# ishine/Prior-DiffuSE

Measured on AMD Instinct MI355X. Metric: enhanced-audio sec/sec (RTF), 6-step fast sampling, B=32, higher is better.
Workload: dtype f16x2; 1 GPU; B=32 x 4 s 16 kHz utterances per GPU, [B,2,401,161] spectrograms, GCRN prior + DiffUNet1 6-step sampling, STFT..ISTFT, seeded random weights; global_batch=32, frames=401, parallelism=batch-shard x1, graph=True, streams_per_gpu=1, batches_in_flight=3

## Files before the change

include/pdse.h:

```cpp
#ifndef PDSE_H
#define PDSE_H
#include <stdint.h>

#ifdef __cplusplus
extern "C" {
#endif

#define PDSE_ABI_VERSION 9

typedef void* pdse_stream_t;

enum pdse_act { PDSE_ACT_NONE = 0, PDSE_ACT_PRELU = 1, PDSE_ACT_ELU = 2, PDSE_ACT_SIGMOID = 3 };

enum pdse_epi {
  PDSE_EPI_LINEAR = 0,
  PDSE_EPI_GLU = 1,
  PDSE_EPI_BIGLU = 2
};

typedef struct pdse_src {
  const float* ptr;
  int64_t sb, sc, st, sf;
  int32_t C;
  int32_t act;
// ... 110 lines not shown
  int32_t reflect_own, pad_;
} pdse_wavprep_desc;

typedef struct pdse_ola_desc {
  const float* frames;
  const float* win2;
  const float* c;
  float* out;
  int32_t B, T, L, n_fft, hop, pad_;
  const int32_t* nframes;
  const int32_t* lens;
} pdse_ola_desc;

typedef struct pdse_qsample_desc {
  const float* label;
  const float* init;
  const float* noise;
  const float* a;
  const float* s;
  float* out;
  int64_t plane;
  int32_t B, mode;
} pdse_qsample_desc;

#define PDSE_MASKLOSS_BLOCKS 32
typedef struct pdse_maskloss_desc {
  const float* esti;
  const float* label;
  const int32_t* frames;
  double* partial;
  float* out;
  int32_t B, C, T, F;
} pdse_maskloss_desc;

typedef struct pdse_sigma_desc {
  const float* init;
  const float* a;
  float* out;
  float* maxbuf;
  int64_t plane;
  int32_t nplanes, pad_;
  const int32_t* valid;
} pdse_sigma_desc;

typedef struct pdse_ln_desc {
  const float* in;
  const float* gamma;
  const float* beta;
  float* out;
  int64_t osb, os_hi, os_lo, os_t;
  int32_t B, T, N, r;
  float eps;
  int32_t blk;
} pdse_ln_desc;

typedef struct pdse_lstm_desc {
  const float* gx;
  const float* whh;
  float* hT;
  float* cst;
  float* y;
  int64_t y_sb, y_st, y_su, y_sg;
  int32_t B, Bp, T, H, G, pad_;
} pdse_lstm_desc;

typedef struct pdse_glstm_desc {
  const float* gx1;
  const float* whh1;
  const float* wih2;
  const float* r2;
  const float* c2;
  const float* whh2;
  float* hT1;
  float* cst1;
  float* hT2;
  float* cst2;
  float* gx2;
  float* part;
  float* y;
  int64_t y_sb, y_st, y_su, y_sg;
  int32_t B, Bp, T, H, G;
  float eps;
  int32_t slices;
  int32_t pad_;
} pdse_glstm_desc;

typedef struct pdse_glstmp_desc {
  const float* gx1;
  const float* w1;
  const float* w2i;
  const float* w2h;
  const float* r2;
  const float* c2;
  unsigned long long* gran;
  int32_t* status;
  float* y;
  int64_t y_sb, y_st, y_su, y_sg;
  int32_t B, Bp, T, H, G;
  float eps;
} pdse_glstmp_desc;


typedef struct pdse_rowln_desc {
  const float* in;
  const float* gamma;
  const float* beta;
  const float* slope;
  float* out;
  int64_t out_sb;
  int32_t B, C, T, F;
  float eps;
  int32_t pad_;
} pdse_rowln_desc;

typedef struct pdse_dense_desc {
  float* D;
  const void* w;
  const float* bias;
  const float* gamma;
  const float* beta;
  const float* slope;
  int32_t B, T, F, G, tpad;
  int32_t g_in, cin;
  int32_t g_out;
  int32_t dil, np;
  float eps;
  int32_t wexp;
} pdse_dense_desc;

typedef struct pdse_rowlnb_desc {
  const float* in;
  const float* gamma;
  const float* beta;
  const float* slope;
  float* out;
  int64_t in_sb, in_sc, in_st;
  int64_t out_sb, out_sg, out_st;
  int32_t B, C, T, F;
  float eps;
  int32_t pad_;
} pdse_rowlnb_desc;

typedef struct pdse_chln_desc {
  const float* in;
  const float* gamma;
  const float* beta;
  float* out;
  int64_t plane;
  int32_t B, C;
  float eps;
  int32_t pad_;
} pdse_chln_desc;

typedef struct pdse_attn_desc {
  const float* qkv;
  float* out;
  int32_t B, T, F, E, heads, axis, pad0_, pad1_;
} pdse_attn_desc;

typedef struct pdse_gru_desc {
  const float* gx;
  const float* whh;
  const float* bhh;
  float* y;
  int32_t B, T, F, H, axis;
  int32_t split;
// ... 333 lines not shown
```

prior-diffuse_amd/_lib.py:

```python
import contextlib
import ctypes as C
import os

_HERE = os.path.dirname(os.path.abspath(__file__))
LIB_PATH = os.environ.get("PDSE_LIB") or os.path.join(_HERE, "libpdse.so")

ABI_VERSION = 9

ACT_NONE, ACT_PRELU, ACT_ELU, ACT_SIGMOID = 0, 1, 2, 3
EPI_LINEAR, EPI_GLU, EPI_BIGLU = 0, 1, 2
EW_DIV, EW_UPDATE, EW_UPDATE_FINAL, EW_COPY, EW_ADD_MUL = 0, 1, 2, 3, 4
(OP_GCONV, OP_TIME, OP_EW, OP_COMPAND, OP_WAVPREP, OP_OLA, OP_SIGMA, OP_LN, OP_LSTM,
 OP_ROWLN, OP_CHLN, OP_ATTN, OP_GRU, OP_GNCOMB, OP_AHAM, OP_QSAMPLE, OP_TRANSPOSE, OP_TCM, OP_CRM, OP_GCRNLAST,
 OP_MASKLOSS, OP_GLSTM, OP_TCM2, OP_BGLU, OP_PLANES, OP_GLSTMP, OP_TCM2S, OP_DENSE, OP_ROWLNB, OP_METRICS, OP_RESAMPLE, OP_RANGE) = range(32)
MASKLOSS_BLOCKS = 32

_fp = C.c_void_p
_i32, _i64, _f32 = C.c_int32, C.c_int64, C.c_float


class Src(C.Structure):
    _fields_ = [("ptr", _fp), ("sb", _i64), ("sc", _i64), ("st", _i64), ("sf", _i64),
                ("C", _i32), ("act", _i32), ("blk", _i32), ("pad_", _i32)]


class GconvDesc(C.Structure):
    _fields_ = [
        ("in0", Src), ("in1", Src),
        ("Tin", _i32), ("Fin", _i32),
        ("padrow", _fp), ("padrow_sb", _i64),
        ("taps", _fp), ("ntaps", _i32), ("sf_in", _i32),
        ("xf_scale0", _fp), ("xf_shift0", _fp), ("xf_scale1", _fp), ("xf_shift1", _fp),
        ("xf_slope0", _f32), ("xf_slope1", _f32), ("xf_mode", _i32), ("cin1", _i32),
        ("w0", _fp), ("w1", _fp), ("ksteps", _i32), ("Cout", _i32),
        ("bias0", _fp), ("bias1", _fp), ("bias0_sb", _i64), ("bias1_sb", _i64),
        ("epi", _i32), ("act", _i32), ("act_slope", _f32), ("C2", _i32),
        ("post_scale", _fp), ("post_shift", _fp),
        ("wlc", _fp), ("wrc", _fp), ("blc", _fp), ("brc", _fp), ("wc2", _fp), ("bc2", _fp),
        ("resid", _fp), ("out", _fp),
        ("out_sb", _i64), ("out_sc_hi", _i64), ("out_sc_lo", _i64), ("out_st", _i64),
        ("out_sf", _i64), ("out_off", _i64),
        ("out_cr", _i32), ("B", _i32), ("Tout", _i32), ("Fout", _i32),
        ("korder", _i32), ("ksteps1", _i32), ("w2", _fp), ("w3", _fp), ("p1mask", _i32), ("Fout1", _i32),
        ("nx_w", _fp), ("nx_bias", _fp * 3), ("nx_add", _fp * 3), ("nx_out", _fp * 3), ("nx_bias_sb", _i64 * 3),
        ("nx_sb", _i64 * 3), ("nx_sc", _i64 * 3), ("nx_st", _i64 * 3), ("nx_sf", _i64 * 3), ("nx_off", _i64 * 3),
        ("nx_n", _i32), ("nx_keep", _i32), ("nx_row0", _i32), ("wexp", _i32),
        ("bias0_t0", _fp), ("bias1_t0", _fp),
        ("tap_dt", _i32 * 12), ("tap_df", _i32 * 12), ("flat", _i32), ("pad_", _i32),
    ]


class TimeDesc(C.Structure):
    _fields_ = [("t", _fp), ("table", _fp), ("p1T", _fp), ("b1", _fp), ("p2T", _fp), ("b2", _fp),
                ("wfT", _fp), ("bf", _fp), ("out", _fp), ("temb", _fp),
                ("B", _i32), ("NF", _i32), ("max_steps", _i32), ("pad_", _i32)]


class EwDesc(C.Structure):
    _fields_ = [("a", _fp), ("b", _fp), ("c", _fp), ("out", _fp), ("n", _i64),
                ("s0", _f32), ("s1", _f32), ("s2", _f32), ("op", _i32)]


class CompandDesc(C.Structure):
    _fields_ = [("in_", _fp), ("out", _fp), ("plane", _i64), ("B", _i32), ("mode", _i32),
                ("out_sb", _i64), ("out_sc", _i64), ("out_st", _i64), ("F", _i32), ("pad_", _i32)]


class WavprepDesc(C.Structure):
    _fields_ = [("wav", _fp), ("xpad", _fp), ("c", _fp), ("lens", _fp),
                ("B", _i32), ("L", _i32), ("pad", _i32), ("normalize", _i32), ("reflect_own", _i32), ("pad_", _i32)]


class OlaDesc(C.Structure):
    _fields_ = [("frames", _fp), ("win2", _fp), ("c", _fp), ("out", _fp),
                ("B", _i32), ("T", _i32), ("L", _i32), ("n_fft", _i32), ("hop", _i32), ("pad_", _i32),
                ("nframes", _fp), ("lens", _fp)]


class SigmaDesc(C.Structure):
    _fields_ = [("init", _fp), ("a", _fp), ("out", _fp), ("maxbuf", _fp), ("plane", _i64),
                ("nplanes", _i32), ("pad_", _i32), ("valid", _fp)]


class LnDesc(C.Structure):
    _fields_ = [("in_", _fp), ("gamma", _fp), ("beta", _fp), ("out", _fp),
                ("osb", _i64), ("os_hi", _i64), ("os_lo", _i64), ("os_t", _i64),
                ("B", _i32), ("T", _i32), ("N", _i32), ("r", _i32), ("eps", _f32), ("blk", _i32)]


class LstmDesc(C.Structure):
    _fields_ = [("gx", _fp), ("whh", _fp), ("hT", _fp), ("cst", _fp), ("y", _fp),
                ("y_sb", _i64), ("y_st", _i64), ("y_su", _i64), ("y_sg", _i64),
                ("B", _i32), ("Bp", _i32), ("T", _i32), ("H", _i32), ("G", _i32), ("pad_", _i32)]


class GlstmDesc(C.Structure):
    _fields_ = [("gx1", _fp), ("whh1", _fp), ("wih2", _fp), ("r2", _fp), ("c2", _fp), ("whh2", _fp),
                ("hT1", _fp), ("cst1", _fp), ("hT2", _fp), ("cst2", _fp), ("gx2", _fp), ("part", _fp), ("y", _fp),
                ("y_sb", _i64), ("y_st", _i64), ("y_su", _i64), ("y_sg", _i64),
                ("B", _i32), ("Bp", _i32), ("T", _i32), ("H", _i32), ("G", _i32), ("eps", _f32), ("slices", _i32), ("pad_", _i32)]


class GlstmpDesc(C.Structure):
    _fields_ = [("gx1", _fp), ("w1", _fp), ("w2i", _fp), ("w2h", _fp), ("r2", _fp), ("c2", _fp), ("gran", _fp), ("status", _fp),
                ("y", _fp), ("y_sb", _i64), ("y_st", _i64), ("y_su", _i64), ("y_sg", _i64),
                ("B", _i32), ("Bp", _i32), ("T", _i32), ("H", _i32), ("G", _i32), ("eps", _f32)]


class RowlnDesc(C.Structure):
    _fields_ = [("in_", _fp), ("gamma", _fp), ("beta", _fp), ("slope", _fp), ("out", _fp), ("out_sb", _i64),
                ("B", _i32), ("C", _i32), ("T", _i32), ("F", _i32), ("eps", _f32), ("pad_", _i32)]


class DenseDesc(C.Structure):
    _fields_ = [("D", _fp), ("w", _fp), ("bias", _fp), ("gamma", _fp), ("beta", _fp), ("slope", _fp),
                ("B", _i32), ("T", _i32), ("F", _i32), ("G", _i32), ("tpad", _i32), ("g_in", _i32), ("cin", _i32), ("g_out", _i32),
                ("dil", _i32), ("np", _i32), ("eps", _f32), ("wexp", _i32)]


class RowlnbDesc(C.Structure):
    _fields_ = [("in_", _fp), ("gamma", _fp), ("beta", _fp), ("slope", _fp), ("out", _fp),
                ("in_sb", _i64), ("in_sc", _i64), ("in_st", _i64), ("out_sb", _i64), ("out_sg", _i64), ("out_st", _i64),
                ("B", _i32), ("C", _i32), ("T", _i32), ("F", _i32), ("eps", _f32), ("pad_", _i32)]


class ChlnDesc(C.Structure):
    _fields_ = [("in_", _fp), ("gamma", _fp), ("beta", _fp), ("out", _fp), ("plane", _i64),
                ("B", _i32), ("C", _i32), ("eps", _f32), ("pad_", _i32)]


class AttnDesc(C.Structure):
    _fields_ = [("qkv", _fp), ("out", _fp), ("B", _i32), ("T", _i32), ("F", _i32), ("E", _i32),
                ("heads", _i32), ("axis", _i32), ("pad0_", _i32), ("pad1_", _i32)]


class GruDesc(C.Structure):
    _fields_ = [("gx", _fp), ("whh", _fp), ("bhh", _fp), ("y", _fp),
                ("B", _i32), ("T", _i32), ("F", _i32), ("H", _i32), ("axis", _i32), ("split", _i32),
                ("x", _fp), ("wih", _fp), ("bih", _fp)]


class GncombDesc(C.Structure):
    _fields_ = [("base", _fp), ("row", _fp), ("col", _fp), ("g_row", _fp), ("b_row", _fp), ("g_col", _fp),
                ("b_col", _fp), ("stats", _fp), ("out", _fp), ("plane", _i64), ("B", _i32), ("C", _i32),
                ("k1", _f32), ("k2", _f32), ("eps", _f32), ("pad_", _i32)]


class AhamDesc(C.Structure):
    _fields_ = [("x", _fp * 4), ("w", _fp), ("means", _fp), ("out", _fp), ("plane", _i64),
                ("B", _i32), ("C", _i32), ("bias", _f32), ("pad_", _i32)]


class QsampleDesc(C.Structure):
    _fields_ = [("label", _fp), ("init", _fp), ("noise", _fp), ("a", _fp), ("s", _fp), ("out", _fp),
                ("plane", _i64), ("B", _i32), ("mode", _i32)]


class MasklossDesc(C.Structure):
    _fields_ = [("esti", _fp), ("label", _fp), ("frames", _fp), ("partial", _fp), ("out", _fp),
                ("B", _i32), ("C", _i32), ("T", _i32), ("F", _i32)]


class TransposeDesc(C.Structure):
    _fields_ = [("in_", _fp), ("out", _fp), ("N", _i32), ("R", _i32), ("Cc", _i32), ("pad_", _i32)]


class TcmDesc(C.Structure):
    _fields_ = [("x", _fp), ("h", _fp), ("x_out", _fp), ("h_out", _fp), ("wbr", _fp), ("bmain", _fp), ("bmask", _fp),
                ("xf", _fp), ("wc2", _fp), ("bc2", _fp), ("xf2", _fp), ("wn1", _fp), ("bn1", _fp),
                ("slope_main", _f32), ("slope_mask", _f32), ("slope2", _f32), ("dil", _i32), ("B", _i32), ("T", _i32),
                ("frames", _fp)]


class Tcm2Desc(C.Structure):
    _fields_ = [("x", _fp), ("x_out", _fp), ("hs", _fp), ("hs_out", _fp), ("wbr", _fp), ("wc2", _fp), ("wn1", _fp),
                ("par", _fp), ("slope2", _f32), ("slope_main_next", _f32), ("slope_mask_next", _f32),
                ("dil", _i32), ("B", _i32), ("T", _i32), ("mode", _i32), ("np", _i32), ("qexp", _i32 * 3),
                ("frames", _fp)]


TCM2S_MAX = 20


# ... 279 lines not shown
```

prior-diffuse_amd/csrc/lstm.hip:

```cpp
#include <hip/hip_runtime.h>
#include <stdio.h>
#include <stdint.h>
#include <stdlib.h>

#include "pdse.h"
#include "pdse_internal.h"

typedef float f32x16 __attribute__((ext_vector_type(16)));

__device__ __forceinline__ float sigm(float x) { return 1.0f / (1.0f + expf(-x)); }

template <int KPW>
__global__ __launch_bounds__(512) void lstm_step_kernel(const pdse_lstm_desc d, const int t, const int pp) {
  __shared__ float red[8][32][33];
  const int lane = threadIdx.x & 63, wave = threadIdx.x >> 6;
  const int col = lane & 31, h = lane >> 5;
  const int slice = blockIdx.x, g = blockIdx.y, bt = blockIdx.z;
  const int H = d.H, Bp = d.Bp, G = d.G;
  const float* hprev = d.hT + ((size_t)(pp * G + g) * H) * Bp + bt * 32;
  float* hnext = d.hT + ((size_t)((pp ^ 1) * G + g) * H) * Bp + bt * 32;
  const int KS = H / 2;
  const float* A = d.whh + ((size_t)(g * (H / 8) + slice) * KS) * 64 + lane;

  f32x16 acc;
#pragma unroll
  for (int r = 0; r < 16; ++r) acc[r] = 0.f;
  if (t > 0) {
    float av[KPW], bv[KPW];
    const int ks0 = wave * KPW;
#pragma unroll
    for (int i = 0; i < KPW; ++i) {
      av[i] = A[(size_t)(ks0 + i) * 64];
      bv[i] = hprev[(size_t)(2 * (ks0 + i) + h) * Bp + col];
    }
    __builtin_amdgcn_sched_barrier(0);
#pragma unroll
    for (int i = 0; i < KPW; ++i) acc = __builtin_amdgcn_mfma_f32_32x32x2f32(av[i], bv[i], acc, 0, 0, 0);
  }
  const int u = threadIdx.x >> 5 & 7, bb = threadIdx.x & 31;
  const int b = bt * 32 + bb;
  const int hu = slice * 8 + u;
  float gxv[4] = {0.f, 0.f, 0.f, 0.f};
  float c_old = 0.f;
  const size_t ci = ((size_t)g * H + hu) * Bp + b;
  if (threadIdx.x < 256) {
#pragma unroll
    for (int q = 0; q < 4; ++q) gxv[q] = d.gx[(((size_t)g * d.T + t) * (4 * H) + (size_t)q * H + hu) * Bp + b];
    if (t > 0) c_old = d.cst[ci];
  }
#pragma unroll
  for (int r = 0; r < 16; ++r) red[wave][(r & 3) + 8 * (r >> 2) + 4 * h][col] = acc[r];
  __syncthreads();
  if (threadIdx.x < 256) {
    float gate[4];
#pragma unroll
    for (int q = 0; q < 4; ++q) {
      const int i = q * 8 + u;
      float s = 0.f;
#pragma unroll
      for (int w = 0; w < 8; ++w) s += red[w][i][bb];
      gate[q] = s + gxv[q];
    }
    const float c = sigm(gate[1]) * c_old + sigm(gate[0]) * tanhf(gate[2]);
    const float hv = sigm(gate[3]) * tanhf(c);
    d.cst[ci] = c;
    hnext[(size_t)hu * Bp + bb] = hv;
    if (b < d.B) d.y[(int64_t)b * d.y_sb + (int64_t)t * d.y_st + (int64_t)hu * d.y_su + (int64_t)g * d.y_sg] = hv;
  }
}

int pdse_lstm_launch(const pdse_lstm_desc* d, hipStream_t s) {
  if (!d || !d->gx || !d->whh || !d->hT || !d->cst || !d->y) {
    pdse_set_error("lstm: null pointer");
    return 1;
  }
  if (d->B <= 0 || d->T <= 0 || d->G <= 0 || d->H != 512 || d->Bp % 32 != 0 || d->Bp < d->B) {
    pdse_set_error("lstm: bad sizes (H == 512 as in gcrn.py:9-16, Bp % 32 == 0, Bp >= B)");
    return 1;
  }
  const dim3 grid(d->H / 8, d->G, d->Bp / 32), block(512);
  for (int t = 0; t < d->T; ++t) hipLaunchKernelGGL(lstm_step_kernel<32>, grid, block, 0, s, *d, t, t & 1);
  return pdse_check_launch("lstm");
}

__device__ __forceinline__ float sigm_g(float x) { return 1.0f / (1.0f + expf(-x)); }

__device__ __forceinline__ size_t hidx(const int u, const int b, const int Bp) {
  return (((size_t)(u >> 3) * 2 + (u & 1)) * Bp + b) * 4 + ((u & 7) >> 1);
}

__device__ long long* g_trace_l = nullptr;
#define LSTAMP(i)                                                                                               \
  do {                                                                                                          \
    if (trace && lane == 0)                                                                                     \
      trace[((((size_t)blockIdx.z * gridDim.y + blockIdx.y) * gridDim.x + blockIdx.x) * 8 + wave) * 8 + (i)] =  \
          (i) == 0 ? wall_clock64() : clock64();                                                                \
  } while (0)

template <int NS>
__global__ __launch_bounds__(512) void glstm_wave_kernel(const pdse_glstm_desc d, const int s, const int stage_mask) {
  extern __shared__ __attribute__((aligned(16))) float lds_[];
  float (*red)[32 * NS][33] = reinterpret_cast<float (*)[32 * NS][33]>(lds_);
  float (*stat)[32][2] = reinterpret_cast<float (*)[32][2]>(lds_ + 8 * 32 * NS * 33);
  float (*gxs)[32][8 * NS] = reinterpret_cast<float (*)[32][8 * NS]>(lds_ + 8 * 32 * NS * 33 + 16 * 32 * 2);
  const int lane = threadIdx.x & 63, wave = threadIdx.x >> 6;
  const int col = lane & 31, h = lane >> 5;
  const int slice = blockIdx.x * NS, g = blockIdx.y;
  const int nbt = d.Bp >> 5;
  const int stage = blockIdx.z / nbt, bt = blockIdx.z - stage * nbt;
  const int t = s - stage;
  if (t < 0 || t >= d.T || !((stage_mask >> stage) & 1)) return;
#ifdef PDSE_DIAG
  long long* const trace = (s == d.T / 2) ? g_trace_l : nullptr;
#else
  long long* const trace = nullptr;
#endif
  LSTAMP(0);
  LSTAMP(1);
  const int H = d.H, Bp = d.Bp, G = d.G;
  const size_t hsz = (size_t)H * Bp;
  const int par = t & 1;

  const float* Aw;
  const float* hsrc0;
  const float* hsrc1;
  int kq0, kq1;
  bool skip = false;
  if (stage == 0) {
    Aw = d.whh1;
    hsrc0 = hsrc1 = d.hT1 + ((size_t)par * G + g) * hsz;
    kq0 = 0, kq1 = 32;
    skip = t == 0;
  } else if (stage == 1) {
    Aw = d.wih2;
    const float* base = d.hT1 + (size_t)((t + 1) & 1) * G * hsz;
    hsrc0 = base, hsrc1 = base + hsz;
    kq0 = kq1 = 32 * g;
  } else {
    Aw = d.whh2;
    hsrc0 = hsrc1 = d.hT2 + ((size_t)par * G + g) * hsz;
    kq0 = 0, kq1 = 32;
    skip = t == 0;
  }
  const float4* A4 = reinterpret_cast<const float4*>(Aw) + ((size_t)(g * (H / 8) + slice) * (H / 8)) * 64 + lane;

  f32x16 acc[NS];
#pragma unroll
  for (int n = 0; n < NS; ++n)
#pragma unroll
    for (int r = 0; r < 16; ++r) acc[n][r] = 0.f;
  if (!skip) {
    float4 av[NS][8], bv[8];
    const int q0 = wave * 8;
    const float* hs = q0 < 32 ? hsrc0 : hsrc1;
    const int kq = (q0 < 32 ? kq0 : kq1) + (q0 & 31);
    const float4* B4 = reinterpret_cast<const float4*>(hs) + ((size_t)kq * 2 + h) * Bp + bt * 32 + col;
    const float k0 = stage == 1 ? hsrc0[(size_t)(bt * 32 + col) * 4] : 0.f;
#pragma unroll
    for (int i = 0; i < 8; ++i) {
#pragma unroll
      for (int n = 0; n < NS; ++n) av[n][i] = A4[((size_t)n * (H / 8) + q0 + i) * 64];
      bv[i] = B4[(size_t)i * 2 * Bp];
    }
    __builtin_amdgcn_sched_barrier(0);
    if (stage == 1) {
#pragma unroll
      for (int i = 0; i < 8; ++i) bv[i].x -= k0, bv[i].y -= k0, bv[i].z -= k0, bv[i].w -= k0;
    }
    if (trace) {
      asm volatile("s_waitcnt vmcnt(0)" ::: "memory");
      LSTAMP(2);
    }
#pragma unroll
    for (int i = 0; i < 8; ++i) {
#pragma unroll
      for (int n = 0; n < NS; ++n) {
        acc[n] = __builtin_amdgcn_mfma_f32_32x32x2f32(av[n][i].x, bv[i].x, acc[n], 0, 0, 0);
        acc[n] = __builtin_amdgcn_mfma_f32_32x32x2f32(av[n][i].y, bv[i].y, acc[n], 0, 0, 0);
        acc[n] = __builtin_amdgcn_mfma_f32_32x32x2f32(av[n][i].z, bv[i].z, acc[n], 0, 0, 0);
        acc[n] = __builtin_amdgcn_mfma_f32_32x32x2f32(av[n][i].w, bv[i].w, acc[n], 0, 0, 0);
      }
    }
  }

  constexpr int NFIN = 256 * NS;
  const int uu = (threadIdx.x >> 5) & (8 * NS - 1), bb = threadIdx.x & 31;
  const int sl = uu >> 3, u = uu & 7;
  const int b = bt * 32 + bb;
  const int hu = (slice + sl) * 8 + u;
  float pre[4] = {0.f, 0.f, 0.f, 0.f};
  float4 gx4 = make_float4(0.f, 0.f, 0.f, 0.f);
  float c_old = 0.f;
  const size_t ci = ((size_t)g * H + hu) * Bp + b;
  if (threadIdx.x < NFIN) {
    if (stage == 0) {
      const int lq = threadIdx.x / (64 * NS), lb = (threadIdx.x / (2 * NS)) & 31, lu = (threadIdx.x & (2 * NS - 1)) * 4;
      gx4 = *reinterpret_cast<const float4*>(d.gx1 + (((size_t)g * d.T + t) * Bp + bt * 32 + lb) * (4 * H) + (size_t)lq * H + slice * 8 + lu);
      if (t > 0) c_old = d.cst1[ci];
    } else if (stage == 2) {
#pragma unroll
      for (int q = 0; q < 4; ++q) pre[q] = d.gx2[(((size_t)par * G + g) * (4 * H) + (size_t)q * H + hu) * Bp + b];
      if (t > 0) c_old = d.cst2[ci];
    }
  }
  float k0e = 0.f;
  if (stage == 1) {
    k0e = hsrc0[(size_t)b * 4];
    const int p = threadIdx.x >> 5;
    const float2* P2 = reinterpret_cast<const float2*>(d.part) + ((size_t)par * G * (H / 8)) * Bp + b;
    float2 pv[8];
    float s1 = 0.f, m2 = 0.f;
#pragma unroll
    for (int e = 0; e < 8; ++e) {
      pv[e] = P2[(size_t)(p * 8 + e) * Bp];
      s1 += pv[e].x;
    }
    const float mp = s1 * (1.0f / 64.0f);
#pragma unroll
    for (int e = 0; e < 8; ++e) {
      const float dv = pv[e].x * 0.125f - mp;
      m2 += pv[e].y + 8.0f * (dv * dv);
    }
    stat[p][bb][0] = s1;
    stat[p][bb][1] = m2;
  }
  LSTAMP(3);
#pragma unroll
  for (int n = 0; n < NS; ++n)
#pragma unroll
    for (int r = 0; r < 16; ++r) red[wave][32 * n + (r & 3) + 8 * (r >> 2) + 4 * h][col] = acc[n][r];
  if (stage == 0 && threadIdx.x < NFIN) {
    const int lq = threadIdx.x / (64 * NS), lb = (threadIdx.x / (2 * NS)) & 31, lu = (threadIdx.x & (2 * NS - 1)) * 4;
    *reinterpret_cast<float4*>(&gxs[lq][lb][lu]) = gx4;
  }
  __syncthreads();
  if (stage == 0 && threadIdx.x < NFIN) {
#pragma unroll
    for (int q = 0; q < 4; ++q) pre[q] = gxs[q][bb][uu];
  }
  LSTAMP(4);
  const bool fin = threadIdx.x < NFIN;
  float gate[4] = {0.f, 0.f, 0.f, 0.f};
  if (fin) {
#pragma unroll
    for (int q = 0; q < 4; ++q) {
      const int i = 32 * sl + q * 8 + u;
      float sum = 0.f;
#pragma unroll
      for (int w = 0; w < 8; ++w) sum += red[w][i][bb];
      gate[q] = sum;
    }
  }
  if (stage == 1) {
    if (!fin) return;
    double s1 = 0.0;
#pragma unroll
    for (int p = 0; p < 16; ++p) s1 += (double)stat[p][bb][0];
    const double n = (double)(G * H);
    const double mu = s1 / n;
    const float muf = (float)mu;
    float m2 = 0.f;
#pragma unroll
    for (int p = 0; p < 16; ++p) {
      const float dv = stat[p][bb][0] * (1.0f / 64.0f) - muf;
      m2 += stat[p][bb][1] + 64.0f * (dv * dv);
    }
    const double var = (double)m2 / n;
    const float rs = (float)(1.0 / sqrt(var + (double)d.eps));
    const float muk = (float)(mu - (double)k0e);
    float* out = d.gx2 + (((size_t)par * G + g) * (4 * H)) * Bp;
#pragma unroll
    for (int q = 0; q < 4; ++q) {
      const size_t row = (size_t)q * H + hu;
      out[row * Bp + b] = rs * (gate[q] - muk * d.r2[(size_t)g * 4 * H + row]) + d.c2[(size_t)g * 4 * H + row];
    }
    return;
  }
  float hv = 0.f;
  if (fin) {
#pragma unroll
    for (int q = 0; q < 4; ++q) gate[q] += pre[q];
    const float c = sigm_g(gate[1]) * c_old + sigm_g(gate[0]) * tanhf(gate[2]);
    hv = sigm_g(gate[3]) * tanhf(c);
    if (stage == 0) {
      d.cst1[ci] = c;
      d.hT1[((size_t)(par ^ 1) * G + g) * hsz + hidx(hu, b, Bp)] = hv;
      stat[uu][bb][0] = hv;
    } else {
      d.cst2[ci] = c;
      d.hT2[((size_t)(par ^ 1) * G + g) * hsz + hidx(hu, b, Bp)] = hv;
      if (b < d.B) d.y[(int64_t)b * d.y_sb + (int64_t)t * d.y_st + (int64_t)hu * d.y_su + (int64_t)g * d.y_sg] = hv;
    }
  }
  LSTAMP(5);
  if (stage != 0) return;
  __syncthreads();
  if (threadIdx.x < 32 * NS) {
    const int ps = threadIdx.x >> 5;
    float v[8];
    float s1 = 0.f, m2 = 0.f;
#pragma unroll
    for (int k = 0; k < 8; ++k) {
      v[k] = stat[8 * ps + k][bb][0];
      s1 += v[k];
    }
    const float m = s1 * 0.125f;
#pragma unroll
    for (int k = 0; k < 8; ++k) {
      const float e = v[k] - m;
      m2 += e * e;
    }
    float2* P2 = reinterpret_cast<float2*>(d.part) + (((size_t)par * G + g) * (H / 8) + slice + ps) * Bp + b;
    *P2 = make_float2(s1, m2);
  }
}


int pdse_glstm_launch(const pdse_glstm_desc* d, hipStream_t s) {
  if (!d || !d->gx1 || !d->whh1 || !d->wih2 || !d->r2 || !d->c2 || !d->whh2 || !d->hT1 || !d->cst1 || !d->hT2 ||
      !d->cst2 || !d->gx2 || !d->part || !d->y) {
    pdse_set_error("glstm: null pointer");
    return 1;
  }
  if (d->B <= 0 || d->T <= 0 || d->G != 2 || d->H != 512 || d->Bp % 32 != 0 || d->Bp < d->B || (d->Bp / 32) * 3 > 65535) {
    pdse_set_error("glstm: bad sizes (H == 512, G == 2 as in gcrn.py:9-16, Bp % 32 == 0, Bp >= B)");
    return 1;
  }
  if (d->slices < 0 || d->slices > 2) {
    pdse_set_error("glstm: slices is 0 / 1 (one slice of 8 units per workgroup) or 2");
    return 1;
  }
  const int NS = d->slices == 2 ? 2 : 1;
  const dim3 grid(d->H / 8 / NS, d->G, 3 * (d->Bp / 32)), block(512);
  const size_t lds = (size_t)(8 * 32 * NS * 33 + 16 * 32 * 2 + 4 * 32 * 8 * NS) * sizeof(float);
  static unsigned long long attr_mask = 0;
  if (NS == 2 && pdse_lds_attr((const void*)glstm_wave_kernel<2>, &attr_mask, "glstm lds attribute")) return 1;
  static const int mask = PDSE_DIAG_ENV("PDSE_GLSTM_MASK") ? atoi(PDSE_DIAG_ENV("PDSE_GLSTM_MASK")) : 7;
  static const bool tracing = PDSE_DIAG_ENV("PDSE_GLSTM_TRACE") != nullptr;
  static long long* tbuf = nullptr;
  const size_t nw = (size_t)grid.x * grid.y * grid.z * 8;
  if (tracing) {
    if (!tbuf) {
      (void)hipMalloc(&tbuf, nw * 64);
      (void)hipMemcpyToSymbol(HIP_SYMBOL(g_trace_l), &tbuf, sizeof(tbuf));
    }
    (void)hipMemsetAsync(tbuf, 0, nw * 64, s);
  }
  for (int st = 0; st < d->T + 2; ++st) {
    if (NS == 2) hipLaunchKernelGGL(glstm_wave_kernel<2>, grid, block, lds, s, *d, st, mask);
    else hipLaunchKernelGGL(glstm_wave_kernel<1>, grid, block, lds, s, *d, st, mask);
  }
  if (tracing) {
    (void)hipStreamSynchronize(s);
    long long* h = (long long*)malloc(nw * 64);
    (void)hipMemcpy(h, tbuf, nw * 64, hipMemcpyDeviceToHost);
    for (int stg = 0; stg < 3; ++stg) {
      double sum[8] = {0};
      long long w0 = -1, w1 = 0;
      size_t n = 0;
      const size_t per = nw / 3;
      for (size_t i = stg * per; i < (stg + 1) * per; ++i) {
        const long long* q = h + i * 8;
        if (!q[0]) continue;
        ++n;
        if (w0 < 0 || q[0] < w0) w0 = q[0];
        if (q[0] > w1) w1 = q[0];
        for (int k = 2; k < 6; ++k) sum[k] += q[k] ? (double)(q[k] - q[1]) : 0.0;
      }
      if (n) fprintf(stderr, "glstm trace stage %d (%zu waves): start spread %.2f us; cycles since wave start: loads landed %.0f, mfma issued %.0f, after barrier %.0f, end %.0f\n",
                     stg, n, (w1 - w0) * 0.01, sum[2] / n, sum[3] / n, sum[4] / n, sum[5] / n);
    }
    free(h);
  }
  return pdse_check_launch("glstm");
}
```

prior-diffuse_amd/nets.py:

```python
import ctypes as C

import numpy as np
import torch

from . import _lib as L
from . import packing as P

F0 = 161
BIG = 1 << 30

TAG_NONE, TAG_EPS_BLOCK, TAG_EPS_CONV1, TAG_TCM, TAG_PRIOR, TAG_LSTM, TAG_SIGNAL, TAG_EW = range(8)


class WeightBank:

    def __init__(self):
        self.items = {}
        self.keep = []
        self.owners = []

    def token(self, obj):
        if obj is None:
            return None
        for i, o in enumerate(self.owners):
# ... 802 lines not shown
                Fin = self._biconvglu_composed(step, src_x, src_i, o, ostr, nx)
            else:
                Fin = self._biconvglu(step, k, src_x, src_i, Fin, o, ostr, H=Hc, do_conv1=(k == 1 or not chained), nx=nx)
            if chained:
                Hc, Hn = Hn, Hc
            src_x, src_i = self.src(o, 64, *nchw(64, T, Fin)), None
        cur, nxt = self.en[4], self.tcm_a
        names = [("TCMs.%d.residual%d" % (i, j + 1), dil) for i in range(3) for j, dil in enumerate((1, 2, 4, 8, 16, 32))]
        if self.force_generic or not self.fused_tcm:
            for p, dil in names:
                self._residual(p, dil, cur, nxt)
                cur, nxt = nxt, (self.tcm_b if nxt is self.tcm_a else self.tcm_a)
        elif self.split_bf16 and self.split_tcm:
            hcur, hnxt = self.tcm_hs
            self._residual_split(None, 1, cur, None, None, hcur, names[0][0], mode=1)
            self._tcm_stack = [] if self.use_tcm_stack else None
            for n, (p, dil) in enumerate(names):
                p_next = names[n + 1][0] if n + 1 < len(names) else None
                self._residual_split(p, dil, cur, nxt, hcur, hnxt, p_next)
                cur, nxt = nxt, (self.tcm_b if nxt is self.tcm_a else self.tcm_a)
                hcur, hnxt = hnxt, hcur
            if self._tcm_stack:
                sd_ = L.Tcm2sDesc()
                for n, blk in enumerate(self._tcm_stack):
                    sd_.blk[n] = blk
                sd_.n = len(self._tcm_stack)
                sd_.flags, sd_.status = self.tcm_flags.data_ptr(), self.tcm_status.data_ptr()
                self.add(sd_, TAG_TCM)
            self._tcm_stack = None
        else:
            hcur, hnxt = self.tcm_h, self.tcm_g
            self._tcm_conv1(names[0][0], cur, hcur)
            for n, (p, dil) in enumerate(names):
                p_next = names[n + 1][0] if n + 1 < len(names) else None
                self._residual_fused(p, dil, cur, nxt, hcur, hnxt, p_next)
                cur, nxt = nxt, (self.tcm_b if nxt is self.tcm_a else self.tcm_a)
                hcur, hnxt = hnxt, hcur
        tcm_out = cur
        if self._plane_stage("dec"):
            self._decoders_planes(step, tcm_out, out)
            return out
        for di, de in enumerate(("de_real", "de_imag")):
            in0 = self.src(tcm_out, 64, 256 * T, 4 * T, 1, T)
            Fin = 4
            Hc, Hn = self.H, self.H2
            for n, k in enumerate((5, 4, 3, 2, 1)):
                skip = self.en[k - 1]
                if k == 5:
                    in1 = self.src(skip, 64, 256 * T, 4 * T, 1, T)
                else:
                    in1 = self.src(skip, 64, *nchw(64, T, self.ENC_F[k]))
                p = "%s.de%d.0" % (de, k)
                if k > 1:
                    o, ooff = self.dec[n & 1], 0
                    fn = lambda Fo: nchw_out(64, T, Fo)
                    bn, pr = "%s.de%d.2" % (de, k), "%s.de%d.3.weight" % (de, k)
                else:
                    o, ooff = out, di * T * F0
                    fn = lambda Fo: nchw_out(2, T, Fo)
                    bn, pr = None, None
                nx = None
                if chained and k > 1:
                    Fo = 2 * (Fin - 1) + 3
                    wn = lambda de=de, k=k: self.w("%s.de%d.0.conv1.weight" % (de, k - 1))[:, :, 0, 0].T[:, :64]
                    nx = dict(keep=False, row0=-1, tiles=[dict(wfn=wn, bias=self.zero32, out=Hn, add=self.Pskip[di][k - 1],
                                                                strides=(32 * T * Fo, T * Fo, Fo, 2))])
                Fin = self._biconvtransglu(step, 5 + 5 * di + n, p, k, in0, in1, Fin, o, fn, bn, pr, out_off=ooff, H=Hc,
                                           do_conv1=(k == 5 or not chained), nx=nx)
                if chained:
                    Hc, Hn = Hn, Hc
                in0 = self.src(o, 64, *nchw(64, T, Fin))
        return out


class GcrnPlan(PlanBase):
    fused_last = True
    fused_glstm = True
    split_bf16 = True
    gemm_planes = 2
    block8 = True
    fuse_phases = True
    flat_proj = True
    persist_lstm = True
    PERSIST_MAX_B = 4
    ENC_C = [2, 16, 32, 64, 128, 256]
    ENC_F = [161, 80, 39, 19, 9, 4]

    def __init__(self, ctx, sd, B, T, plan=None, split_bf16=None, exclusive=False, planes=None):
        if split_bf16 is not None:
            self.split_bf16 = bool(split_bf16)
        if planes is not None:
            if planes not in (1, 2, 3) or (planes in (1, 2) and not self.split_bf16):
                raise ValueError("planes is 3 (bf16x3), 2 (f16x2) or 1 (bf16 mode); the one- and two-plane forms run on the GEMM kernels (split_bf16)")
            self.gemm_planes = int(planes)
        self.persist = bool(self.persist_lstm and self.fused_glstm and exclusive and B <= self.PERSIST_MAX_B and not self.force_generic)
        self.exclusive = bool(exclusive)
        super().__init__(ctx, plan, ns=(ctx.bank.token(sd), self.fused_last, self.fused_glstm, self.split_bf16, self.block8, self.persist,
                                        self.gemm_planes))
        self.sd, self.B, self.T = sd, B, T
        a = ctx.alloc
        self.Bp = Bp = (B + 31) // 32 * 32
        self.status = None
        self.x = a(B, 2, T, F0)
        self.out = a(B, 2, T, F0)
        self.e = [a(B, self.ENC_C[i + 1], T, self.ENC_F[i + 1]) for i in range(5)]
        self.gx = a(2, T, 2048, Bp, zero=True)
        self.hT = a(2, 2, 512, Bp, zero=True)
        self.cst = a(2, 512, Bp, zero=True)
        self.y = a(B, T, 1024)
        if self.persist:
            bq = 1 << (B - 1).bit_length()
            self.gran = torch.zeros(4 * 1024 * bq, dtype=torch.int64, device=ctx.device)
            self.status = torch.zeros(4, dtype=torch.int32, device=ctx.device)
            ctx.keep += [self.gran, self.status]
        elif self.fused_glstm and not self.force_generic:
            self.hT2, self.cst2 = a(2, 2, 512, Bp, zero=True), a(2, 512, Bp, zero=True)
            self.gx2, self.part = a(2, 2, 2048, Bp, zero=True), a(2, 2, 64, Bp, 2, zero=True)
        else:
            self.yn = a(B, 1024, T)
        self.glstm = a(B, 256, T, 4)
        self.d = [a(B, 128, T, 9), a(B, 64, T, 19), a(B, 32, T, 39), a(B, 16, T, 80), a(B, 1, T, 161)]
        for i, t_ in enumerate(self.e):
            self.named("gcrn.e%d" % (i + 1), t_)
        self.named("gcrn.glstm", self.glstm)
        for i, t_ in enumerate(self.d[:4]):
            self.named("gcrn.d%d" % (5 - i), t_)
        self.named("gcrn.x", self.x)

    def w(self, k):
        return P._np(self.sd[k])

    def _nchw(self, t, blocked):
        if blocked and self.split_bf16 and not self.force_generic and self.block8:
            B, C_, T, F = t.shape
            return t.view(B, C_ // 8, T, F, 8).permute(0, 1, 4, 2, 3).reshape(B, C_, T, F)
        return t

    def enc_out(self, k):
        return self._nchw(self.e[k - 1], k >= 2)

    def glstm_out(self):
        return self._nchw(self.glstm, True)

    def _lstm_proj(self, layer, proj, gx_lay):
        B, T, Bp = self.B, self.T, self.Bp
        for g in range(2):
            p = "glstm.%s.%d." % (layer, g)
            in0, Tin, Fin, taps, wk_fn, Tout, Fout, ost, osf = proj(g)
            self.gconv(in0=in0, Tin=Tin, Fin=Fin, taps=taps, sf_in=1, Cout=2048,
                       W=lambda p=p, wk_fn=wk_fn: dict(wk0=wk_fn(self.w(p + "weight_ih_l0")),
                                                       bias0=self.w(p + "bias_ih_l0") + self.w(p + "bias_hh_l0")),
                       out=self.gx, out_strides=gx_lay + (0, ost, osf), out_off=g * T * 2048 * Bp, B=B, Tout=Tout, Fout=Fout,
                       tag=TAG_PRIOR, label=p + "ih", s3g=self.split_bf16,
                       flat=self.flat_proj and Fout == 1 and len(taps) * in0.C <= 512)

    def _lstm_layer(self, layer, xproj_src_fn, y_su, y_sg):
        B, T, Bp = self.B, self.T, self.Bp
        self._lstm_proj(layer, xproj_src_fn, (1, Bp))

        def pack_whh():
            return P.pack_lstm_whh([self.w("glstm.%s.%d.weight_hh_l0" % (layer, g)) for g in range(2)])

        d = L.LstmDesc()
        d.gx, d.whh = self.gx.data_ptr(), self.upw(layer + ".whh", pack_whh).data_ptr()
        d.hT, d.cst, d.y = self.hT.data_ptr(), self.cst.data_ptr(), self.y.data_ptr()
        d.y_sb, d.y_st, d.y_su, d.y_sg = T * 1024, 1024, y_su, y_sg
        d.B, d.Bp, d.T, d.H, d.G = B, Bp, T, 512, 2
        self.add(d, TAG_LSTM)

    def _glstm_natural(self):
        per = lambda key: [self.w("glstm.%s" % (key % g)) for g in range(2)]
        return (per("lstm_list1.%d.weight_hh_l0"), per("lstm_list2.%d.weight_ih_l0"), per("lstm_list2.%d.bias_ih_l0"),
                per("lstm_list2.%d.bias_hh_l0"), per("lstm_list2.%d.weight_hh_l0"), self.w("glstm.ln1.weight"), self.w("glstm.ln1.bias"))

    def _glstm_wavefront(self, proj1):
        B, T, Bp = self.B, self.T, self.Bp
        self._lstm_proj("lstm_list1", proj1, (2048, 1))
        d = L.GlstmDesc()
        self.apply(d, self.fields("glstm.wavefront", lambda: P.pack_glstm_wavefront(*self._glstm_natural())))
        d.gx1, d.gx2, d.part = self.gx.data_ptr(), self.gx2.data_ptr(), self.part.data_ptr()
        d.hT1, d.cst1, d.hT2, d.cst2 = self.hT.data_ptr(), self.cst.data_ptr(), self.hT2.data_ptr(), self.cst2.data_ptr()
        d.y, d.y_sb, d.y_st, d.y_su, d.y_sg = self.y.data_ptr(), T * 1024, 1024, 1, 512
        d.B, d.Bp, d.T, d.H, d.G, d.eps = B, Bp, T, 512, 2, 1e-5
        d.slices = 2 if self.exclusive else 1
        self.add(d, TAG_LSTM)

    def _glstm_persistent(self, proj1):
        B, T, Bp = self.B, self.T, self.Bp
        self._lstm_proj("lstm_list1", proj1, (2048, 1))
        d = L.GlstmpDesc()
        self.apply(d, self.fields("glstm.persistent", lambda: P.pack_glstm_persistent(*self._glstm_natural())))
        d.gx1, d.gran, d.status = self.gx.data_ptr(), self.gran.data_ptr(), self.status.data_ptr()
        d.y, d.y_sb, d.y_st, d.y_su, d.y_sg = self.y.data_ptr(), T * 1024, 1024, 1, 512
        d.B, d.Bp, d.T, d.H, d.G, d.eps = B, Bp, T, 512, 2, 1e-5
        self.add(d, TAG_LSTM)

    def _ln(self, name, out_t, osb, os_hi, os_lo, os_t, r, blk=0):
        d = L.LnDesc()
        d.blk = blk
        d.in_, d.out = self.y.data_ptr(), out_t.data_ptr()
        d.gamma = self.upw(name + ".g", lambda: self.w(name + ".weight")).data_ptr()
        d.beta = self.upw(name + ".b", lambda: self.w(name + ".bias")).data_ptr()
        d.osb, d.os_hi, d.os_lo, d.os_t = osb, os_hi, os_lo, os_t
        d.B, d.T, d.N, d.r, d.eps = self.B, self.T, 1024, r, 1e-5
        self.add(d, TAG_PRIOR)

    def build(self, x=None, out=None):
        B, T, Bp = self.B, self.T, self.Bp
        x = self.x if x is None else x
        out = self.out if out is None else out
        blk = self.split_bf16 and not self.force_generic and self.block8

        def lay(k_is_blocked, C_, Fq):
            if k_is_blocked:
                return nc8(C_, T, Fq), nc8_out(C_, T, Fq), 8
            return nchw(C_, T, Fq), nchw_out(C_, T, Fq), 1

        src = self.src(x, 2, *nchw(2, T, F0))
        e_lay = [lay(blk and k >= 2, self.ENC_C[k], self.ENC_F[k]) for k in range(1, 6)]
        for k in range(1, 6):
            ci, co, Fin, Fout = self.ENC_C[k - 1], self.ENC_C[k], self.ENC_F[k - 1], self.ENC_F[k]
            kk, taps = P.conv_taps(1, 3, 0)
            p = "conv%d" % k
            ist, ost_, ocr = e_lay[k - 1]
            self.gconv(in0=src, Tin=T, Fin=Fin, taps=taps, sf_in=2, Cout=co, epi=L.EPI_GLU, act=L.ACT_ELU,
                       W=lambda p=p, k=k, kk=kk: dict(wk0=P.conv_kmat(self.sd[p + ".conv1.weight"], kk),
                                                      wk1=P.conv_kmat(self.sd[p + ".conv2.weight"], kk),
                                                      bias0=self.w(p + ".conv1.bias"), bias1=self.w(p + ".conv2.bias"),
                                                      post=P.bn_fold(self.sd, "bn%d" % k)),
                       out=self.e[k - 1], out_strides=ost_, out_cr=ocr, B=B, Tout=T, Fout=Fout, tag=TAG_PRIOR, label=p,
                       s3g=self.split_bf16)
            src = self.src(self.e[k - 1], co, *ist, blk=8 if ocr == 8 else 0)

        def proj1(g):
            wk = lambda Wih: np.concatenate([Wih[:, f::4].T for f in range(4)], axis=0)
            s = self.src(self.e[4], 128, *e_lay[4][0], off=128 * g * T * 4, blk=8 if blk else 0)
            return s, T, 4, [(0, f) for f in range(4)], wk, T, 1, 2048 * Bp, 0

        if self.persist:
            self._glstm_persistent(proj1)
        elif self.fused_glstm and not self.force_generic:
            self._glstm_wavefront(proj1)
        else:
            self._lstm_layer("lstm_list1", proj1, y_su=2, y_sg=1)
            self._ln("glstm.ln1", self.yn, 1024 * T, T, 0, 1, 1)

            def proj2(g):
                s = self.src(self.yn, 512, 1024 * T, T, 0, 1, off=512 * g * T)
                return s, 1, T, [(0, 0)], (lambda Wih: Wih.T), 1, T, 0, 2048 * Bp

            self._lstm_layer("lstm_list2", proj2, y_su=1, y_sg=512)
        if blk:
            self._ln("glstm.ln2", self.glstm, 256 * T * 4, T * 4 * 8, 8, 4 * 8, 4, blk=8)
        else:
            self._ln("glstm.ln2", self.glstm, 256 * T * 4, T * 4, 1, 4, 4)

        dec = [(5, 512, 128), (4, 256, 64), (3, 128, 32), (2, 64, 16), (1, 32, 1)]
        for br in (1, 2):
            in0 = self.src(self.glstm, 256, *(nc8(256, T, 4) if blk else nchw(256, T, 4)), blk=8 if blk else 0)
            in1 = self.src(self.e[4], 256, *e_lay[4][0], blk=8 if blk else 0)
            Fin = 4
            for n, (k, ci, co) in enumerate(dec):
                p = "conv%d_t_%d" % (k, br)
                Fout = 2 * (Fin - 1) + 3 + (1 if k == 2 else 0)
                if k == 1 and self.fused_last and not self.force_generic:
                    g = L.GcrnLastDesc()
                    self.apply(g, self.fields(p + ".last", lambda p=p, br=br: P.gcrn_last_fields(self.sd, p, br)))
# ... 475 lines not shown
```

Before: 9629 audio_s/s.

## Chunk grouped-LSTM layer-2 input projection into batched per-chunk kernel launches

Replaces the three-stage per-timestep wavefront (LSTM1, LN+projection, LSTM2) with a two-stage wavefront where LSTM2 lags LSTM1 by tc+1 steps. The layer-2 input projection with its layer norm now runs in a separate kernel once per chunk of 32 timesteps, reading ring buffers sized 2*tc. The aim is to take the projection stage off the sequential per-step critical path and process several timesteps per launch. It costs larger hT/gx2/part ring buffers, extra launches at chunk boundaries, and a longer pipeline tail at the end of the sequence.

New measurement: 9726 audio_s/s, median of 6. +1.0%, better.

```diff
diff --git a/include/pdse.h b/include/pdse.h
--- a/include/pdse.h
+++ b/include/pdse.h
@@ -216,6 +216,8 @@
   int32_t B, Bp, T, H, G;
   float eps;
   int32_t slices;
+  int32_t tc;
+  int32_t lag;
   int32_t pad_;
 } pdse_glstm_desc;
 
diff --git a/prior-diffuse_amd/_lib.py b/prior-diffuse_amd/_lib.py
--- a/prior-diffuse_amd/_lib.py
+++ b/prior-diffuse_amd/_lib.py
@@ -98,7 +98,8 @@
     _fields_ = [("gx1", _fp), ("whh1", _fp), ("wih2", _fp), ("r2", _fp), ("c2", _fp), ("whh2", _fp),
                 ("hT1", _fp), ("cst1", _fp), ("hT2", _fp), ("cst2", _fp), ("gx2", _fp), ("part", _fp), ("y", _fp),
                 ("y_sb", _i64), ("y_st", _i64), ("y_su", _i64), ("y_sg", _i64),
-                ("B", _i32), ("Bp", _i32), ("T", _i32), ("H", _i32), ("G", _i32), ("eps", _f32), ("slices", _i32), ("pad_", _i32)]
+                ("B", _i32), ("Bp", _i32), ("T", _i32), ("H", _i32), ("G", _i32), ("eps", _f32), ("slices", _i32), ("tc", _i32), ("lag", _i32),
+                ("pad_", _i32)]
 
 
 class GlstmpDesc(C.Structure):
diff --git a/prior-diffuse_amd/csrc/lstm.hip b/prior-diffuse_amd/csrc/lstm.hip
--- a/prior-diffuse_amd/csrc/lstm.hip
+++ b/prior-diffuse_amd/csrc/lstm.hip
@@ -97,7 +97,7 @@
           (i) == 0 ? wall_clock64() : clock64();                                                                \
   } while (0)
 
-template <int NS>
+template <int NS, bool CH>
 __global__ __launch_bounds__(512) void glstm_wave_kernel(const pdse_glstm_desc d, const int s, const int stage_mask) {
   extern __shared__ __attribute__((aligned(16))) float lds_[];
   float (*red)[32 * NS][33] = reinterpret_cast<float (*)[32 * NS][33]>(lds_);
@@ -107,8 +107,9 @@
   const int col = lane & 31, h = lane >> 5;
   const int slice = blockIdx.x * NS, g = blockIdx.y;
   const int nbt = d.Bp >> 5;
-  const int stage = blockIdx.z / nbt, bt = blockIdx.z - stage * nbt;
-  const int t = s - stage;
+  const int zs = blockIdx.z / nbt, bt = blockIdx.z - zs * nbt;
+  const int stage = CH ? 2 * zs : zs;
+  const int t = s - (CH ? (stage ? d.lag : 0) : stage);
   if (t < 0 || t >= d.T || !((stage_mask >> stage) & 1)) return;
 #ifdef PDSE_DIAG
   long long* const trace = (s == d.T / 2) ? g_trace_l : nullptr;
@@ -120,6 +121,9 @@
   const int H = d.H, Bp = d.Bp, G = d.G;
   const size_t hsz = (size_t)H * Bp;
   const int par = t & 1;
+  const int R = CH ? 2 * d.tc : 2;
+  const int r1 = CH ? t % R : par;
+  const int w1 = CH ? (t + 1) % R : par ^ 1;
 
   const float* Aw;
   const float* hsrc0;
@@ -128,10 +132,10 @@
   bool skip = false;
   if (stage == 0) {
     Aw = d.whh1;
-    hsrc0 = hsrc1 = d.hT1 + ((size_t)par * G + g) * hsz;
+    hsrc0 = hsrc1 = d.hT1 + ((size_t)r1 * G + g) * hsz;
     kq0 = 0, kq1 = 32;
     skip = t == 0;
-  } else if (stage == 1) {
+  } else if (!CH && stage == 1) {
     Aw = d.wih2;
     const float* base = d.hT1 + (size_t)((t + 1) & 1) * G * hsz;
     hsrc0 = base, hsrc1 = base + hsz;
@@ -155,7 +159,7 @@
     const float* hs = q0 < 32 ? hsrc0 : hsrc1;
     const int kq = (q0 < 32 ? kq0 : kq1) + (q0 & 31);
     const float4* B4 = reinterpret_cast<const float4*>(hs) + ((size_t)kq * 2 + h) * Bp + bt * 32 + col;
-    const float k0 = stage == 1 ? hsrc0[(size_t)(bt * 32 + col) * 4] : 0.f;
+    const float k0 = !CH && stage == 1 ? hsrc0[(size_t)(bt * 32 + col) * 4] : 0.f;
 #pragma unroll
     for (int i = 0; i < 8; ++i) {
 #pragma unroll
@@ -163,7 +167,7 @@
       bv[i] = B4[(size_t)i * 2 * Bp];
     }
     __builtin_amdgcn_sched_barrier(0);
-    if (stage == 1) {
+    if (!CH && stage == 1) {
 #pragma unroll
       for (int i = 0; i < 8; ++i) bv[i].x -= k0, bv[i].y -= k0, bv[i].z -= k0, bv[i].w -= k0;
     }
@@ -199,12 +203,12 @@
       if (t > 0) c_old = d.cst1[ci];
     } else if (stage == 2) {
 #pragma unroll
-      for (int q = 0; q < 4; ++q) pre[q] = d.gx2[(((size_t)par * G + g) * (4 * H) + (size_t)q * H + hu) * Bp + b];
+      for (int q = 0; q < 4; ++q) pre[q] = d.gx2[(((size_t)r1 * G + g) * (4 * H) + (size_t)q * H + hu) * Bp + b];
       if (t > 0) c_old = d.cst2[ci];
     }
   }
   float k0e = 0.f;
-  if (stage == 1) {
+  if (!CH && stage == 1) {
     k0e = hsrc0[(size_t)b * 4];
     const int p = threadIdx.x >> 5;
     const float2* P2 = reinterpret_cast<const float2*>(d.part) + ((size_t)par * G * (H / 8)) * Bp + b;
@@ -251,7 +255,7 @@
       gate[q] = sum;
     }
   }
-  if (stage == 1) {
+  if (!CH && stage == 1) {
     if (!fin) return;
     double s1 = 0.0;
 #pragma unroll
@@ -284,7 +288,7 @@
     hv = sigm_g(gate[3]) * tanhf(c);
     if (stage == 0) {
       d.cst1[ci] = c;
-      d.hT1[((size_t)(par ^ 1) * G + g) * hsz + hidx(hu, b, Bp)] = hv;
+      d.hT1[((size_t)w1 * G + g) * hsz + hidx(hu, b, Bp)] = hv;
       stat[uu][bb][0] = hv;
     } else {
       d.cst2[ci] = c;
@@ -310,11 +314,154 @@
       const float e = v[k] - m;
       m2 += e * e;
     }
-    float2* P2 = reinterpret_cast<float2*>(d.part) + (((size_t)par * G + g) * (H / 8) + slice + ps) * Bp + b;
+    float2* P2 = reinterpret_cast<float2*>(d.part) + (((size_t)r1 * G + g) * (H / 8) + slice + ps) * Bp + b;
     *P2 = make_float2(s1, m2);
   }
 }
 
+constexpr int PROJ_BUF = 8 * 32 * 33 + 16 * 32 * 2;
+__global__ __launch_bounds__(512) void glstm_proj_kernel(const pdse_glstm_desc d, const int t0, const int nf, const int FS) {
+  extern __shared__ __attribute__((aligned(16))) float lds_[];
+  const int lane = threadIdx.x & 63, wave = threadIdx.x >> 6;
+  const int col = lane & 31, h = lane >> 5;
+  const int slice = blockIdx.x, g = blockIdx.y;
+  const int nbt = d.Bp >> 5;
+  const int fs = blockIdx.z / nbt, bt = blockIdx.z - fs * nbt;
+  const int per = (nf + FS - 1) / FS;
+  const int f0 = fs * per, f1 = min(nf, f0 + per);
+  if (f0 >= f1) return;
+  const int H = d.H, Bp = d.Bp, G = d.G;
+  const size_t hsz = (size_t)H * Bp;
+  const int R = 2 * d.tc;
+
+  const int q0 = wave * 8;
+  const size_t srcoff = (size_t)(q0 >> 5) * hsz;
+  const int kq = 32 * g + (q0 & 31);
+  const size_t boff = ((size_t)kq * 2 + h) * Bp + bt * 32 + col;
+  const float4* A4 = reinterpret_cast<const float4*>(d.wih2) + ((size_t)(g * (H / 8) + slice) * (H / 8)) * 64 + lane;
+  float4 av[8], bv[8], bn[8];
+#pragma unroll
+  for (int i = 0; i < 8; ++i) av[i] = A4[(size_t)(q0 + i) * 64];
+
+  const int uu = (threadIdx.x >> 5) & 7, bb = threadIdx.x & 31;
+  const int b = bt * 32 + bb;
+  const int hu = slice * 8 + uu;
+  const int p = threadIdx.x >> 5;
+  const bool fin = threadIdx.x < 256;
+  float r2v[4], c2v[4];
+#pragma unroll
+  for (int q = 0; q < 4; ++q) {
+    r2v[q] = d.r2[(size_t)g * 4 * H + (size_t)q * H + hu];
+    c2v[q] = d.c2[(size_t)g * 4 * H + (size_t)q * H + hu];
+  }
+
+  const float* base = d.hT1 + (size_t)((t0 + f0 + 1) % R) * G * hsz;
+  float k0 = base[(size_t)(bt * 32 + col) * 4], k0n = 0.f;
+  {
+    const float4* B4 = reinterpret_cast<const float4*>(base + srcoff) + boff;
+#pragma unroll
+    for (int i = 0; i < 8; ++i) bv[i] = B4[(size_t)i * 2 * Bp];
+  }
+  for (int f = f0; f < f1; ++f) {
+    const int t = t0 + f;
+    float* const buf = lds_ + ((f - f0) & 1) * PROJ_BUF;
+    float (*red)[32][33] = reinterpret_cast<float (*)[32][33]>(buf);
+    float (*stat)[32][2] = reinterpret_cast<float (*)[32][2]>(buf + 8 * 32 * 33);
+    const float k0e = base[(size_t)b * 4];
+    const float2* P2 = reinterpret_cast<const float2*>(d.part) + ((size_t)(t % R) * G * (H / 8)) * Bp + b;
+    float2 pv[8];
+#pragma unroll
+    for (int e = 0; e < 8; ++e) pv[e] = P2[(size_t)(p * 8 + e) * Bp];
+    if (f + 1 < f1) {
+      base = d.hT1 + (size_t)((t + 2) % R) * G * hsz;
+      k0n = base[(size_t)(bt * 32 + col) * 4];
+      const float4* B4 = reinterpret_cast<const float4*>(base + srcoff) + boff;
+#pragma unroll
+      for (int i = 0; i < 8; ++i) bn[i] = B4[(size_t)i * 2 * Bp];
+    }
+    __builtin_amdgcn_sched_barrier(0);
+#pragma unroll
+    for (int i = 0; i < 8; ++i) bv[i].x -= k0, bv[i].y -= k0, bv[i].z -= k0, bv[i].w -= k0;
+    f32x16 acc;
+#pragma unroll
+    for (int r = 0; r < 16; ++r) acc[r] = 0.f;
+#pragma unroll
+    for (int i = 0; i < 8; ++i) {
+      acc = __builtin_amdgcn_mfma_f32_32x32x2f32(av[i].x, bv[i].x, acc, 0, 0, 0);
+      acc = __builtin_amdgcn_mfma_f32_32x32x2f32(av[i].y, bv[i].y, acc, 0, 0, 0);
+      acc = __builtin_amdgcn_mfma_f32_32x32x2f32(av[i].z, bv[i].z, acc, 0, 0, 0);
+      acc = __builtin_amdgcn_mfma_f32_32x32x2f32(av[i].w, bv[i].w, acc, 0, 0, 0);
+    }
+    {
+      float s1 = 0.f, m2 = 0.f;
+#pragma unroll
+      for (int e = 0; e < 8; ++e) s1 += pv[e].x;
+      const float mp = s1 * (1.0f / 64.0f);
+#pragma unroll
+      for (int e = 0; e < 8; ++e) {
+        const float dv = pv[e].x * 0.125f - mp;
+        m2 += pv[e].y + 8.0f * (dv * dv);
+      }
+      stat[p][bb][0] = s1;
+      stat[p][bb][1] = m2;
+    }
+#pragma unroll
+    for (int r = 0; r < 16; ++r) red[wave][(r & 3) + 8 * (r >> 2) + 4 * h][col] = acc[r];
+    __syncthreads();
+    if (fin) {
+      float gate[4];
+#pragma unroll
+      for (int q = 0; q < 4; ++q) {
+        float sum = 0.f;
+#pragma unroll
+        for (int w = 0; w < 8; ++w) sum += red[w][q * 8 + uu][bb];
+        gate[q] = sum;
+      }
+      double s1 = 0.0;
+#pragma unroll
+      for (int pp = 0; pp < 16; ++pp) s1 += (double)stat[pp][bb][0];
+      const double n = (double)(G * H);
+      const double mu = s1 / n;
+      const float muf = (float)mu;
+      float m2 = 0.f;
+#pragma unroll
+      for (int pp = 0; pp < 16; ++pp) {
+        const float dv = stat[pp][bb][0] * (1.0f / 64.0f) - muf;
+        m2 += stat[pp][bb][1] + 64.0f * (dv * dv);
+      }
+      const double var = (double)m2 / n;
+      const float rs = (float)(1.0 / sqrt(var + (double)d.eps));
+      const float muk = (float)(mu - (double)k0e);
+      float* out = d.gx2 + (((size_t)(t % R) * G + g) * (4 * H)) * Bp;
+#pragma unroll
+      for (int q = 0; q < 4; ++q) out[((size_t)q * H + hu) * Bp + b] = rs * (gate[q] - muk * r2v[q]) + c2v[q];
+    }
+    k0 = k0n;
+#pragma unroll
+    for (int i = 0; i < 8; ++i) bv[i] = bn[i];
+  }
+}
+
+static int glstm_chunk_launch(const pdse_glstm_desc* d, hipStream_t s, const int mask) {
+  const int NS = d->slices == 2 ? 2 : 1, TC = d->tc, T = d->T, nbt = d->Bp / 32;
+  const dim3 grid(d->H / 8 / NS, d->G, 2 * nbt), block(512);
+  const size_t lds = (size_t)(8 * 32 * NS * 33 + 16 * 32 * 2 + 4 * 32 * 8 * NS) * sizeof(float);
+  const size_t plds = (size_t)2 * PROJ_BUF * sizeof(float);
+  static unsigned long long attr_wave = 0, attr_proj = 0;
+  if (NS == 2 && pdse_lds_attr((const void*)glstm_wave_kernel<2, true>, &attr_wave, "glstm lds attribute")) return 1;
+  if (pdse_lds_attr((const void*)glstm_proj_kernel, &attr_proj, "glstm projection lds attribute")) return 1;
+  for (int st = 0; st < T + TC + 1; ++st) {
+    if (st > 0 && st <= T && (st % TC == 0 || st == T) && (mask & 2)) {
+      const int t0 = (st - 1) / TC * TC, nf = st - t0;
+      const int FS = min(nf, nbt == 1 ? 2 : 1);
+      hipLaunchKernelGGL(glstm_proj_kernel, dim3(d->H / 8, d->G, nbt * FS), block, plds, s, *d, t0, nf, FS);
+    }
+    if (st >= T && st < d->lag) continue;
+    if (NS == 2) hipLaunchKernelGGL((glstm_wave_kernel<2, true>), grid, block, lds, s, *d, st, mask);
+    else hipLaunchKernelGGL((glstm_wave_kernel<1, true>), grid, block, lds, s, *d, st, mask);
+  }
+  return pdse_check_launch("glstm");
+}
 
 int pdse_glstm_launch(const pdse_glstm_desc* d, hipStream_t s) {
   if (!d || !d->gx1 || !d->whh1 || !d->wih2 || !d->r2 || !d->c2 || !d->whh2 || !d->hT1 || !d->cst1 || !d->hT2 ||
@@ -322,6 +469,14 @@
     pdse_set_error("glstm: null pointer");
     return 1;
   }
+  if (d->tc < 0 || (d->tc == 0 && d->lag != 0)) {
+    pdse_set_error("glstm: chunked form needs tc >= 1 (tc == 0 and lag == 0: the three-stage wavefront)");
+    return 1;
+  }
+  if (d->tc > 0 && (d->lag != d->tc + 1 || d->tc > 4096)) {
+    pdse_set_error("glstm: lag must be tc + 1 (tc <= 4096)");
+    return 1;
+  }
   if (d->B <= 0 || d->T <= 0 || d->G != 2 || d->H != 512 || d->Bp % 32 != 0 || d->Bp < d->B || (d->Bp / 32) * 3 > 65535) {
     pdse_set_error("glstm: bad sizes (H == 512, G == 2 as in gcrn.py:9-16, Bp % 32 == 0, Bp >= B)");
     return 1;
@@ -330,12 +485,13 @@
     pdse_set_error("glstm: slices is 0 / 1 (one slice of 8 units per workgroup) or 2");
     return 1;
   }
+  static const int mask = PDSE_DIAG_ENV("PDSE_GLSTM_MASK") ? atoi(PDSE_DIAG_ENV("PDSE_GLSTM_MASK")) : 7;
+  if (d->tc > 0) return glstm_chunk_launch(d, s, mask);
   const int NS = d->slices == 2 ? 2 : 1;
   const dim3 grid(d->H / 8 / NS, d->G, 3 * (d->Bp / 32)), block(512);
   const size_t lds = (size_t)(8 * 32 * NS * 33 + 16 * 32 * 2 + 4 * 32 * 8 * NS) * sizeof(float);
   static unsigned long long attr_mask = 0;
-  if (NS == 2 && pdse_lds_attr((const void*)glstm_wave_kernel<2>, &attr_mask, "glstm lds attribute")) return 1;
-  static const int mask = PDSE_DIAG_ENV("PDSE_GLSTM_MASK") ? atoi(PDSE_DIAG_ENV("PDSE_GLSTM_MASK")) : 7;
+  if (NS == 2 && pdse_lds_attr((const void*)glstm_wave_kernel<2, false>, &attr_mask, "glstm lds attribute")) return 1;
   static const bool tracing = PDSE_DIAG_ENV("PDSE_GLSTM_TRACE") != nullptr;
   static long long* tbuf = nullptr;
   const size_t nw = (size_t)grid.x * grid.y * grid.z * 8;
@@ -347,8 +503,8 @@
     (void)hipMemsetAsync(tbuf, 0, nw * 64, s);
   }
   for (int st = 0; st < d->T + 2; ++st) {
-    if (NS == 2) hipLaunchKernelGGL(glstm_wave_kernel<2>, grid, block, lds, s, *d, st, mask);
-    else hipLaunchKernelGGL(glstm_wave_kernel<1>, grid, block, lds, s, *d, st, mask);
+    if (NS == 2) hipLaunchKernelGGL((glstm_wave_kernel<2, false>), grid, block, lds, s, *d, st, mask);
+    else hipLaunchKernelGGL((glstm_wave_kernel<1, false>), grid, block, lds, s, *d, st, mask);
   }
   if (tracing) {
     (void)hipStreamSynchronize(s);
diff --git a/prior-diffuse_amd/nets.py b/prior-diffuse_amd/nets.py
--- a/prior-diffuse_amd/nets.py
+++ b/prior-diffuse_amd/nets.py
@@ -908,6 +908,8 @@
     fuse_phases = True
     flat_proj = True
     persist_lstm = True
+    chunk_proj = True
+    CHUNK_TC = 32
     PERSIST_MAX_B = 4
     ENC_C = [2, 16, 32, 64, 128, 256]
     ENC_F = [161, 80, 39, 19, 9, 4]
@@ -921,6 +923,8 @@
             self.gemm_planes = int(planes)
         self.persist = bool(self.persist_lstm and self.fused_glstm and exclusive and B <= self.PERSIST_MAX_B and not self.force_generic)
         self.exclusive = bool(exclusive)
+        self.chunk = bool(self.chunk_proj and self.fused_glstm and not exclusive and not self.persist and not self.force_generic
+                          and T >= 2 * self.CHUNK_TC)
         super().__init__(ctx, plan, ns=(ctx.bank.token(sd), self.fused_last, self.fused_glstm, self.split_bf16, self.block8, self.persist,
                                         self.gemm_planes))
         self.sd, self.B, self.T = sd, B, T
@@ -931,7 +935,8 @@
         self.out = a(B, 2, T, F0)
         self.e = [a(B, self.ENC_C[i + 1], T, self.ENC_F[i + 1]) for i in range(5)]
         self.gx = a(2, T, 2048, Bp, zero=True)
-        self.hT = a(2, 2, 512, Bp, zero=True)
+        R = 2 * self.CHUNK_TC if self.chunk else 2
+        self.hT = a(R, 2, 512, Bp, zero=True)
         self.cst = a(2, 512, Bp, zero=True)
         self.y = a(B, T, 1024)
         if self.persist:
@@ -941,7 +946,7 @@
             ctx.keep += [self.gran, self.status]
         elif self.fused_glstm and not self.force_generic:
             self.hT2, self.cst2 = a(2, 2, 512, Bp, zero=True), a(2, 512, Bp, zero=True)
-            self.gx2, self.part = a(2, 2, 2048, Bp, zero=True), a(2, 2, 64, Bp, 2, zero=True)
+            self.gx2, self.part = a(R, 2, 2048, Bp, zero=True), a(R, 2, 64, Bp, 2, zero=True)
         else:
             self.yn = a(B, 1024, T)
         self.glstm = a(B, 256, T, 4)
@@ -1009,6 +1014,8 @@
         d.y, d.y_sb, d.y_st, d.y_su, d.y_sg = self.y.data_ptr(), T * 1024, 1024, 1, 512
         d.B, d.Bp, d.T, d.H, d.G, d.eps = B, Bp, T, 512, 2, 1e-5
         d.slices = 2 if self.exclusive else 1
+        if self.chunk:
+            d.tc, d.lag = self.CHUNK_TC, self.CHUNK_TC + 1
         self.add(d, TAG_LSTM)
 
     def _glstm_persistent(self, proj1):
```
